# yhenon/pixeltable-yolox

Measured on AMD Instinct MI355X. Metric: images/sec (fwd+NMS) YOLOX-s 640×640 bf16 @1/2/4/8 MI355X; box mAP parity, higher is better.
Workload: dtype bf16

## Files before the change

### pixeltable-yolox_amd/csrc/conv_ws.hip

```cpp
#include "conv_common.hpp"
#include "lds_dma.hpp"

#ifndef YXH_WS_PROBE
#define YXH_WS_PROBE 0
#endif

#ifndef YXH_WS_PD8
#define YXH_WS_PD8 0
#endif

#ifndef YXH_WS_NPIN
#define YXH_WS_NPIN 48
#endif

#ifndef YXH_WS_ACT_CT
#define YXH_WS_ACT_CT 1
#endif

namespace yxh {

namespace {

template <typename T, int CR>
__device__ __forceinline__ uint4 ws_weight_padk(const ConvParams& p, int n_first, int tap, int kb, int lane) {
    const int frow = lane & 15, fq = lane >> 4;
    const int ch = kb * 32 + fq * 8;
    if (ch >= CR) return make_uint4(0, 0, 0, 0);
    const int n = min(n_first + frow, p.cout - 1);
    return *(const uint4*)((const T*)p.w + ((long long)n * 9 + tap) * CR + ch);
}

__device__ __forceinline__ void pin_agpr(uint4& v) {
    typedef unsigned u32x4v __attribute__((ext_vector_type(4)));
    u32x4v t = {v.x, v.y, v.z, v.w};
    asm volatile("" : "+a"(t));
    v = make_uint4(t.x, t.y, t.z, t.w);
}

constexpr int ws_ps(int c16, int s) {
    return s == 1 ? c16 + (6 - c16 % 4) % 4 : (c16 % 2 ? c16 : c16 + 1);
}
constexpr int ws_hxp(int tx, int s) {
    const int hx = (tx - 1) * s + 3;
    if (tx % 16 == 0) return hx;
    int h = hx;
    while (h % 8 != tx % 8) ++h;
    return h;
}

}

template <typename T, int CIN, int S, int TX, int TY, int TN, int WN, int WK, int WM, int BPC, bool F1, int PGN = 0,
          int PGC = 0, int PGH = 0, int CR = CIN, bool A32 = false>
__global__ __launch_bounds__(64 * WN * WK * WM, BPC) void conv_ws(ConvParams p, int tiles_x, int tiles_y,
                                                                 int ntiles, int ntn, int nwork) {
    static_assert(sizeof(T) == 2, "16-bit operands");
    constexpr int NW = WN * WK * WM;
    constexpr int NCB = CIN / 32, WCB = NCB / WK;
    constexpr int WTN = TN / WN, FR = WTN / 16;
    constexpr int TM = TX * TY, WTM = TM / WM, FC = WTM / 16;
    constexpr int HX = (TX - 1) * S + 3, HY = (TY - 1) * S + 3, HXP = ws_hxp(TX, S);
    constexpr int C16 = CIN / 8, PS = ws_ps(C16, S), PSB = PS * 16;
    constexpr int SLOTS = HY * HXP * PS, LOADS = (SLOTS + 63) / 64, GB = (LOADS + NW - 1) / NW;
    constexpr int RBYTES = WK > 1 ? WN * WM * FR * FC * (WK - 1) * 1024 : 0;
    constexpr bool PG = PGN > 0, HP = PGH > 0, PGY = PG || HP;
    constexpr int RS = TN / 8 + 1, RSLOTS = (S == 1 || PGY) ? TM * RS : 0;
    constexpr int RLOADS = (RSLOTS + 63) / 64, GR = (RLOADS + NW - 1) / NW, RTB = RLOADS * 1024;
    constexpr int NRING = 3;
    constexpr int XS = PGC / 8 + 1, XSLOTS = PG && PGC > 0 ? TM * XS : 0;
    constexpr int XLOADS = (XSLOTS + 63) / 64, GX = (XLOADS + NW - 1) / NW, XTB = XLOADS * 1024;
    constexpr int K2 = TN + PGC, KB2 = K2 / 32;
    constexpr int WN2 = PG ? (NW < PGN / 16 ? NW : PGN / 16) : 1, WM2 = NW / WN2;
    constexpr int NF2 = PG ? PGN / 16 / WN2 : 1, PF2 = TM / 16 / WM2;
    static_assert(!PG || (!F1 && TN % 32 == 0 && PGC % 32 == 0 && PGN % (16 * WN2) == 0 &&
                          NW % WN2 == 0 && (TM / 16) % WM2 == 0), "post-conv tile");
    static_assert(!HP || (!PG && !F1 && S == 1 && TN % 32 == 0), "head-form tile");
    constexpr int HROWS = HP ? PGH * 16 : 0, HBYTES_W = HROWS * RS * 16 + HROWS * 4;
    constexpr int NG = CIN / 32, R1 = NW / NG, NPA = (HY * HXP + 15) / 16;
    constexpr int HBYTES = LOADS * 1024;
    constexpr int XOFF = 2 * HBYTES + RBYTES + NRING * RTB;
    constexpr int TOFF = XOFF + 3 * XTB;
    constexpr int HWOFF = TOFF + (F1 ? HBYTES : 0);
    constexpr int SMEM = HWOFF + HBYTES_W;
    static_assert(!F1 || (S == 1 && NW % NG == 0), "fused Bottleneck tile");
    constexpr int FCO = (FC + WK - 1) / WK;
    constexpr int NS = WCB * 9;
    constexpr int PD = YXH_WS_PD8 && FR * FC >= 8 ? YXH_WS_PD8 : FR * FC >= 8 ? 1 : FR * FC >= 4 ? 2 : 3;
    static_assert(NCB % WK == 0 && WTN % 16 == 0 && WTM % 16 == 0 && TM % (16 * WM) == 0, "tile");
    static_assert(FR * 9 * WCB * 4 <= (NW == 4 && BPC == 1 ? 288 : 160), "weights must stay in VGPRs");
    static_assert(SMEM <= 160 * 1024 && SMEM * BPC <= 160 * 1024, "LDS (BPC blocks per CU must fit)");
    constexpr int NPIN = !F1 && FR * 9 * WCB * 4 > 160 ? YXH_WS_NPIN : 0;
    __shared__ __attribute__((aligned(16))) char smem[SMEM];

    const int tid = threadIdx.x, lane = tid & 63;
    const int wave = __builtin_amdgcn_readfirstlane(tid >> 6);
    const int wn = wave % WN, wk = (wave / WN) % WK, wm = wave / (WN * WK);
    const int frow = lane & 15, fq = lane >> 4;
    const int bid = dma::xcd_remap(blockIdx.x, gridDim.x);
    const int nt = bid % ntn, worker = bid / ntn;
    const int n0 = nt * TN;
    const int tile = worker;
    if (tile >= ntiles) return;

    const int cin_ = p.cin, cout = p.cout, in_w = p.in_w, in_h = p.in_h, scs = p.scs[0];
    const int OH = p.out_h, OW = p.out_w, ohw = p.ohw;
    (void)cin_;

    uint32_t boff[FC];
#pragma unroll
    for (int j = 0; j < FC; ++j) {
        const int pl = (wm * FC + j) * 16 + frow;
        const int ty = pl / TX, tx = pl - ty * TX;
        boff[j] = (uint32_t)((ty * S * HXP + tx * S) * PSB + (wk * WCB * 4 + fq) * 16);
    }

    const uint32_t lds0 = dma::lds_addr(smem);
    const uint32_t bytes = (uint32_t)((long long)in_h * in_w * scs * 2);
    const int gsrc = p.grp2 && n0 >= cout / 2 ? CR : 0;

    int hrel[GB], hyx[GB];
#pragma unroll
    for (int i = 0; i < GB; ++i) {
        const int L = wave + NW * i;
        const int s = 64 * L + lane;
        const int hp = s / PS, c16 = s - hp * PS;
        const int hy = hp / HXP, hx = hp - hy * HXP;
        const bool st = L < LOADS && s < SLOTS && c16 < CR / 8 && hx < HX;
        hyx[i] = st ? (hy | (hx << 16)) : 0x7fff7fff;
        hrel[i] = ((hy * in_w + hx) * scs + c16 * 8) * 2;
    }

    struct TileC { int b, oy0, ox0; };
    const unsigned txy = (unsigned)(tiles_x * tiles_y);
    auto coords = [&](int t) -> TileC {
        const unsigned b = (unsigned)t / txy, r = (unsigned)t - b * txy;
        const unsigned ty = r / (unsigned)tiles_x, tx = r - ty * (unsigned)tiles_x;
        return TileC{(int)b, (int)ty * TY, (int)tx * TX};
    };

    auto issue_halo = [&](const TileC& c, int kb) {
        const int iy0 = c.oy0 * S - 1, ix0 = c.ox0 * S - 1;
        const int base = (iy0 * in_w + ix0) * scs * 2;
        const dma::u32x4 rsrc = dma::srd((const T*)p.sptr[0] + (long long)c.b * p.sbs[0] + gsrc, bytes);
#pragma unroll
        for (int i = 0; i < GB; ++i) {
            const int L = wave + NW * i;
            if (LOADS % NW == 0 || i + 1 < GB || L < LOADS) {
                const int iy = iy0 + (hyx[i] & 0xffff), ix = ix0 + (hyx[i] >> 16);
                const bool ok = (unsigned)iy < (unsigned)in_h && (unsigned)ix < (unsigned)in_w;
                const uint32_t voff = ok ? (uint32_t)(base + hrel[i]) : dma::kOob;
                dma::load16(rsrc, voff, 0u, __builtin_amdgcn_readfirstlane(lds0 + (uint32_t)(kb * HBYTES + L * 1024)));
            }
        }
    };

    const bool silu = p.act == YXH_ACT_SILU;
    const bool has_res = p.res != nullptr;
    const bool pg_store = PG && p.pg_store;
    const uint32_t dbytes = (uint32_t)((long long)ohw * p.dst_cs * (A32 ? 4 : 2));
    const uint32_t rbytes = (uint32_t)((long long)ohw * p.res_cs * 2);
    const int dcs = p.dst_cs, rcs = p.res_cs;
    const uint32_t res_lds = lds0 + (uint32_t)(2 * HBYTES + RBYTES);

    int rgeo[GR > 0 ? GR : 1];
#pragma unroll
    for (int i = 0; i < GR; ++i) {
        const int L = wave + NW * i;
        const int sl = 64 * L + lane;
        const int pl = sl / RS, ch = sl - pl * RS;
        const int ty = pl / TX, tx = pl - ty * TX;
        const bool st = L < RLOADS && sl < RSLOTS && ch < TN / 8 && n0 + ch * 8 < cout;
        rgeo[i] = st ? (ty | (tx << 10) | (ch << 20)) : -1;
    }
    auto issue_res = [&](const TileC& c, int slot) {
        if constexpr (GR > 0) {
            const dma::u32x4 rsrc = dma::srd((const T*)p.res + (long long)c.b * p.res_bs, rbytes);
#pragma unroll
            for (int i = 0; i < GR; ++i) {
                const int L = wave + NW * i;
                if (RLOADS % NW == 0 || i + 1 < GR || L < RLOADS) {
                    const int g = rgeo[i];
                    const int oy = c.oy0 + (g & 1023), ox = c.ox0 + ((g >> 10) & 1023);
                    const bool ok = g >= 0 && oy < OH && ox < OW;
                    const uint32_t voff = ok ? (uint32_t)(((oy * OW + ox) * rcs + n0 + (g >> 20) * 8) * 2) : dma::kOob;
                    dma::load16(rsrc, voff, 0u, __builtin_amdgcn_readfirstlane(res_lds + (uint32_t)(slot * RTB + L * 1024)));
                }
            }
        }
    };

    int xgeo[GX > 0 ? GX : 1];
#pragma unroll
    for (int i = 0; i < GX; ++i) {
        const int L = wave + NW * i;
        const int sl = 64 * L + lane;
        const int pl = sl / XS, ch = sl - pl * XS;
        const int ty = pl / TX, tx = pl - ty * TX;
        const bool st = L < XLOADS && sl < XSLOTS && ch < PGC / 8;
        xgeo[i] = st ? (ty | (tx << 10) | (ch << 20)) : -1;
    }
    auto issue_x2 = [&](const TileC& c, int slot) {
        if constexpr (GX > 0) {
            const dma::u32x4 xsrc =
                dma::srd((const T*)p.pgs + (long long)c.b * p.pgs_bs, (uint32_t)((long long)ohw * p.pgs_cs * 2));
#pragma unroll
            for (int i = 0; i < GX; ++i) {
                const int L = wave + NW * i;
                if (XLOADS % NW == 0 || i + 1 < GX || L < XLOADS) {
                    const int g = xgeo[i];
                    const int oy = c.oy0 + (g & 1023), ox = c.ox0 + ((g >> 10) & 1023);
                    const bool ok = g >= 0 && oy < OH && ox < OW;
                    const uint32_t voff = ok ? (uint32_t)(((oy * OW + ox) * p.pgs_cs + (g >> 20) * 8) * 2) : dma::kOob;
                    dma::load16(xsrc, voff, 0u,
                                __builtin_amdgcn_readfirstlane(lds0 + (uint32_t)(XOFF + slot * XTB + L * 1024)));
                }
            }
        }
    };

    TileC cur = coords(tile), cnext{0, 0, 0}, prev{0, 0, 0}, prev2{0, 0, 0};
    issue_halo(cur, 0);
    if (!PGY && has_res) issue_res(cur, 0);
    if (tile + nwork < ntiles) {
        cnext = coords(tile + nwork);
        issue_halo(cnext, 1);
        if (!PGY && has_res) issue_res(cnext, 1);
    }

    const bool hgrp1 = HP && n0 >= cout / 2;
    const int hrows = HP ? (hgrp1 ? p.pg_cout2 : p.pg_cout) : 0;

    uint4 a1[F1 ? 2 : 1][F1 ? NG : 1];
    float b1[2][4];
    if constexpr (F1) {
        const T* w1 = (const T*)p.pw1;
        const int g = wave % NG;
#pragma unroll
        for (int i = 0; i < 2; ++i) {
#pragma unroll
            for (int cb = 0; cb < NG; ++cb)
                a1[i][cb] = *(const uint4*)(w1 + (g * 32 + i * 16 + frow) * CIN + cb * 32 + fq * 8);
#pragma unroll
            for (int r = 0; r < 4; ++r) b1[i][r] = p.pb1[g * 32 + i * 16 + fq * 4 + r];
        }
    }

    uint4 a[FR][9][WCB];
#pragma unroll
    for (int c = 0; c < WCB; ++c)
#pragma unroll
        for (int tap = 0; tap < 9; ++tap)
#pragma unroll
            for (int i = 0; i < FR; ++i)
                a[i][tap][c] = CR == CIN ? ws_weight<T>(p, n0 + wn * WTN + i * 16, tap, 9, CIN, wk * WCB + c, lane)
                                         : ws_weight_padk<T, CR>(p, n0 + wn * WTN + i * 16, tap, wk * WCB + c, lane);
    float bias[FR][4];
#pragma unroll
    for (int i = 0; i < FR; ++i) {
        const int n = n0 + wn * WTN + i * 16 + fq * 4;
#pragma unroll
        for (int r = 0; r < 4; ++r) bias[i][r] = n + r < cout ? p.bias[n + r] : 0.0f;
    }


    const int wn2 = wave % WN2, wm2 = wave / WN2;
    uint4 a2[PG ? NF2 : 1][PG ? KB2 : 1];
    float b2[PG ? NF2 : 1][4];
    if constexpr (PG) {
        const T* w2 = (const T*)p.pgw;
#pragma unroll
        for (int f = 0; f < NF2; ++f) {
            const int n = (wn2 * NF2 + f) * 16;
#pragma unroll
            for (int kb = 0; kb < KB2; ++kb) a2[f][kb] = *(const uint4*)(w2 + (long long)(n + frow) * K2 + kb * 32 + fq * 8);
#pragma unroll
            for (int r = 0; r < 4; ++r) b2[f][r] = p.pgb[n + fq * 4 + r];
        }
    }

    typedef uint32_t u32x2 __attribute__((ext_vector_type(2)));
    struct EpiCtx { __amdgpu_buffer_rsrc_t dsrd; const char* rl; TileC c; };
    auto epi_ctx = [&](const TileC c, const int k) -> EpiCtx {
        char* db = (char*)p.dst + (long long)c.b * p.dst_bs * (A32 ? 4 : 2);
        return EpiCtx{__builtin_amdgcn_make_buffer_rsrc((void*)db, (short)0, (int)dbytes, 0x00020000),
                      smem + 2 * HBYTES + RBYTES + (k % NRING) * RTB, c};
    };
    auto epi_piece = [&](const EpiCtx& e, const f32x4 (&ap)[FR][FCO], const int o, const int i, auto act_c) {
        constexpr int AC = decltype(act_c)::value;
        const int j = wk + WK * o;
        const int pl = (wm * FC + j) * 16 + frow;
        const int ty = pl / TX, tx = pl - ty * TX;
        const int oy = e.c.oy0 + ty, ox = e.c.ox0 + tx;
        const int nl = wn * WTN + i * 16 + fq * 4, n = n0 + nl;
        const bool ok = j < FC && oy < OH && ox < OW && n < cout;
        if constexpr (A32) {
            typedef uint32_t u32x4 __attribute__((ext_vector_type(4)));
            const int od4 = ok ? ((oy * OW + ox) * dcs + n) * 4 : (int)dma::kOob;
            f32x4 v = ap[i][o] + f32x4{bias[i][0], bias[i][1], bias[i][2], bias[i][3]};
            if (p.accum) v += __builtin_bit_cast(f32x4, __builtin_amdgcn_raw_buffer_load_b128(e.dsrd, od4, 0, 0));
            __builtin_amdgcn_raw_buffer_store_b128(__builtin_bit_cast(u32x4, v), e.dsrd, od4, 0, 0);
            return;
        }
        const int od = ok ? ((oy * OW + ox) * dcs + n) * 2 : (int)dma::kOob;
        u32x2 rv = {0u, 0u};
        if constexpr (GR > 0) rv = *(const u32x2*)(e.rl + (pl * RS + (nl >> 3)) * 16 + (nl & 7) * 2);
        T rt[4];
        __builtin_memcpy(rt, &rv, 8);
        const f32x4 x = ap[i][o] + f32x4{bias[i][0], bias[i][1], bias[i][2], bias[i][3]};
        f32x4 v;
        if constexpr (AC == 1) v = yxh::silu4(x);
        else if constexpr (AC == 2) v = x;
        else v = silu ? yxh::silu4(x) : x;
        if (has_res) v = v + f32x4{to_f32(rt[0]), to_f32(rt[1]), to_f32(rt[2]), to_f32(rt[3])};
        T t[4] = {from_f32<T>(v[0]), from_f32<T>(v[1]), from_f32<T>(v[2]), from_f32<T>(v[3])};
        u32x2 u;
        __builtin_memcpy(&u, t, 8);
        if constexpr (PGY) {
            *(u32x2*)(e.rl + (pl * RS + (nl >> 3)) * 16 + (nl & 7) * 2) = u;
            if (PG && pg_store) __builtin_amdgcn_raw_buffer_store_b64(u, e.dsrd, od, 0, 0);
        } else if (!(YXH_WS_PROBE & 1) || p.act == 12345) {
            __builtin_amdgcn_raw_buffer_store_b64(u, e.dsrd, od, 0, 0);
        }
    };
    auto epilogue = [&](const TileC c, const int k, const f32x4 (&ap)[FR][FCO], auto act_c) {
        const EpiCtx e = epi_ctx(c, k);
#pragma unroll
        for (int o = 0; o < FCO; ++o)
#pragma unroll
            for (int i = 0; i < FR; ++i) epi_piece(e, ap, o, i, act_c);
    };

    struct PostCtx { __amdgpu_buffer_rsrc_t srd; const char* ys; const char* xs; TileC c; };
    auto post_ctx = [&](const TileC c, const int k) -> PostCtx {
        PostCtx q;
        q.c = c;
        q.ys = smem + 2 * HBYTES + RBYTES + (k % NRING) * RTB;
        q.xs = smem + XOFF + (k % 3) * XTB;
        const int es = HP ? 4 : 2;
        q.srd = __builtin_amdgcn_make_buffer_rsrc((void*)((char*)p.pgd + (long long)c.b * p.pgd_bs * es), (short)0,
                                                  (int)((long long)ohw * p.pgd_cs * es), 0x00020000);
        return q;
    };
    constexpr int HPF = (TM / 16 + NW - 1) / NW;
    constexpr int NPU = PG ? PF2 * NF2 : HP ? HPF * PGH : 0;
    constexpr int KBP = PG ? KB2 : HP ? 2 * (TN / 32) : 1;
    constexpr bool SPLIT = PG;
    constexpr int SP = SPLIT && NS / (NPU + 1) > 1 ? NS / (NPU + 1) : 1;
    auto post_skip = [&](const int u) -> bool {
        if constexpr (HP) {
            const int pf = wave + NW * (u / PGH), f = u - PGH * (u / PGH);
            return pf >= TM / 16 || f >= (hgrp1 ? 1 : PGH);
        }
        return false;
    };
    auto post_load = [&](const PostCtx& q, const int u, uint4 (&ob)[KBP]) {
        if constexpr (PG) {
            const int pf = u / NF2;
            const int pl = (wm2 * PF2 + pf) * 16 + frow;
#pragma unroll
            for (int kb = 0; kb < KB2; ++kb)
                ob[kb] = kb < TN / 32 ? *(const uint4*)(q.ys + (pl * RS + kb * 4 + fq) * 16)
                                      : *(const uint4*)(q.xs + (pl * XS + (kb - TN / 32) * 4 + fq) * 16);
        } else if constexpr (HP) {
            if (post_skip(u)) return;
            const int pf = wave + NW * (u / PGH), f = u - PGH * (u / PGH);
            const char* wl = smem + HWOFF;
#pragma unroll
            for (int kb = 0; kb < TN / 32; ++kb) {
                ob[2 * kb] = *(const uint4*)(q.ys + ((pf * 16 + frow) * RS + kb * 4 + fq) * 16);
                ob[2 * kb + 1] = *(const uint4*)(wl + ((f * 16 + frow) * RS + kb * 4 + fq) * 16);
            }
        }
    };
    auto post_math = [&](const PostCtx& q, const int u, const uint4 (&ob)[KBP]) {
        if constexpr (PG) {
            const int pf = u / NF2, f = u - NF2 * (u / NF2);
            const int pl = (wm2 * PF2 + pf) * 16 + frow;
            f32x4 z = f32x4{0.f, 0.f, 0.f, 0.f};
#pragma unroll
            for (int kb = 0; kb < KB2; ++kb) Mma<T>::run(z, a2[f][kb], ob[kb]);
            const int ty = pl / TX, tx = pl - ty * TX;
            const int oy = q.c.oy0 + ty, ox = q.c.ox0 + tx;
            const int n = (wn2 * NF2 + f) * 16 + fq * 4;
            const f32x4 zs = yxh::silu4(z + f32x4{b2[f][0], b2[f][1], b2[f][2], b2[f][3]});
            T t[4] = {from_f32<T>(zs[0]), from_f32<T>(zs[1]), from_f32<T>(zs[2]), from_f32<T>(zs[3])};
            u32x2 uv;
            __builtin_memcpy(&uv, t, 8);
            const int od = oy < OH && ox < OW ? ((oy * OW + ox) * p.pgd_cs + n) * 2 : (int)dma::kOob;
            __builtin_amdgcn_raw_buffer_store_b64(uv, q.srd, od, 0, 0);
        } else if constexpr (HP) {
            if (post_skip(u)) return;
            const int pf = wave + NW * (u / PGH), f = u - PGH * (u / PGH);
            const float* bl = (const float*)(smem + HWOFF + HROWS * RS * 16);
            f32x4 z = f32x4{0.f, 0.f, 0.f, 0.f};
#pragma unroll
            for (int kb = 0; kb < TN / 32; ++kb) Mma<T>::run(z, ob[2 * kb], ob[2 * kb + 1]);
            const float st = p.pg_stride;
            const int ch = f * 16 + frow;
            const float bch = bl[ch];
#pragma unroll
            for (int r = 0; r < 4; ++r) {
                const int pl = pf * 16 + fq * 4 + r;
                const int ty = pl / TX, tx = pl - ty * TX;
                const int oy = q.c.oy0 + ty, ox = q.c.ox0 + tx;
                const bool okp = oy < OH && ox < OW;
                const int rowo = (oy * OW + ox) * p.pgd_cs + (hgrp1 ? 0 : 5);
                float v = z[r] + bch;
                if (hgrp1) {
                    if (ch < 2) v = (v + (float)(ch == 0 ? ox : oy)) * st;
                    else if (ch < 4) v = __builtin_amdgcn_exp2f(v * 1.4426950408889634f) * st;
                    else v = __builtin_amdgcn_rcpf(1.0f + __builtin_amdgcn_exp2f(-v * 1.4426950408889634f));
                } else {
                    v = __builtin_amdgcn_rcpf(1.0f + __builtin_amdgcn_exp2f(-v * 1.4426950408889634f));
                }
                __builtin_amdgcn_raw_buffer_store_b32(__float_as_uint(v), q.srd,
                                                      okp && ch < hrows ? (rowo + ch) * 4 : (int)dma::kOob, 0, 0);
            }
        }
    };
    auto post_piece = [&](const PostCtx& q, const int u) {
        uint4 ob[KBP];
        post_load(q, u, ob);
        post_math(q, u, ob);
    };
    auto post_all = [&](const PostCtx& q) {
#pragma unroll
        for (int u = 0; u < NPU; ++u) post_piece(q, u);
    };

    f32x4 accp[FR][FCO];
    constexpr int NP = FR * FCO;

    auto tile_step = [&](const TileC cur, const int tile, const int k, TileC& cnext, const TileC prev,
                         const TileC prev2, auto epi, auto post, auto first, auto act_c) -> int {
        constexpr bool EPI = decltype(epi)::value;
        constexpr bool POST = decltype(post)::value && PGY;
        constexpr bool FIRST = decltype(first)::value;
        const int kb = k & 1;
        const int next = tile + nwork;
        if constexpr (FIRST) dma::wait_vm<(FR * 9 * WCB < 63 ? FR * 9 * WCB : 63)>();
        else dma::wait_vm<0>();
        dma::barrier();
        if (next < ntiles) {
            cnext = coords(next);
            if (!FIRST && !(YXH_WS_PROBE & 2)) {
                issue_halo(cnext, kb ^ 1);
                if (!PGY && has_res) issue_res(cnext, (k + 1) % 3);
            }
        }
        if constexpr (PGY) {
            if (has_res) issue_res(cur, k % 3);
            issue_x2(cur, k % 3);
        }

        if constexpr (F1) {
            const char* hx_img = smem + kb * HBYTES;
            char* timg = smem + TOFF;
            const int g = wave % NG;
            for (int fa = wave / NG; fa < NPA; fa += R1) {
                const int hq = fa * 16 + frow;
                const int hpr = min(hq, HY * HXP - 1);
                f32x4 t2[2] = {f32x4{0.f, 0.f, 0.f, 0.f}, f32x4{0.f, 0.f, 0.f, 0.f}};
#pragma unroll
                for (int cb = 0; cb < NG; ++cb) {
                    const uint4 xb = *(const uint4*)(hx_img + hpr * PSB + (cb * 4 + fq) * 16);
                    Mma<T>::run(t2[0], a1[0][cb], xb);
                    Mma<T>::run(t2[1], a1[1][cb], xb);
                }
                const int hy = hq / HXP, hx = hq - hy * HXP;
                const int iy = cur.oy0 - 1 + hy, ix = cur.ox0 - 1 + hx;
                const bool valid = hx < HX && (unsigned)iy < (unsigned)in_h && (unsigned)ix < (unsigned)in_w;
#pragma unroll
                for (int i = 0; i < 2; ++i) {
                    T t[4];
#pragma unroll
                    for (int q = 0; q < 4; ++q) {
                        const float x = t2[i][q] + b1[i][q];
                        t[q] = from_f32<T>(valid ? (silu ? yxh::silu<false>(x) : x) : 0.0f);
                    }
                    u32x2 u;
                    __builtin_memcpy(&u, t, 8);
                    if (hq < HY * HXP) *(u32x2*)(timg + hq * PSB + (g * 32 + i * 16 + fq * 4) * 2) = u;
                }
            }
            dma::barrier();
        }

        f32x4 acc[FR][FC];
#pragma unroll
        for (int i = 0; i < FR; ++i)
#pragma unroll
            for (int j = 0; j < FC; ++j) acc[i][j] = f32x4{0.f, 0.f, 0.f, 0.f};
        const char* hb = F1 ? smem + TOFF : smem + kb * HBYTES;
        uint4 bf[PD + 1][FC];
        auto load_b = [&](int s, uint4 (&d)[FC]) {
            const int c = s / 9, tap = s - 9 * (s / 9);
            const int ky = tap / 3, kx = tap - 3 * (tap / 3);
            const int so = (ky * HXP + kx) * PSB + c * 64;
#pragma unroll
            for (int j = 0; j < FC; ++j) d[j] = *(const uint4*)(hb + boff[j] + so);
        };
#pragma unroll
        for (int q = 0; q < PD; ++q)
            if (q < NS) load_b(q, bf[q]);
        __builtin_amdgcn_sched_group_barrier(0x100, FC * (PD < NS ? PD : NS), 0);
        EpiCtx e{};
        if constexpr (EPI) e = epi_ctx(prev, k - 1);
        PostCtx pc{};
        if constexpr (POST) pc = post_ctx(prev2, k - 2);
        uint4 pob[KBP];
#pragma unroll
        for (int s = 0; s < NS; ++s) {
            if (s + PD < NS) load_b(s + PD, bf[(s + PD) % (PD + 1)]);
            const int c = s / 9, tap = s - 9 * (s / 9);
            if constexpr (FIRST && NPIN > 0) {
#pragma unroll
                for (int i = 0; i < FR; ++i)
                    if ((c * 9 + tap) * FR + i < NPIN) pin_agpr(a[i][tap][c]);
            }
            if constexpr (HP) {
#pragma unroll
                for (int i = 0; i < FR; ++i)
#pragma unroll
                    for (int j = 0; j < FC; ++j) Mma<T>::run(acc[i][j], a[i][tap][c], bf[s % (PD + 1)][j]);
            } else {
#pragma unroll
                for (int j = 0; j < FC; ++j)
#pragma unroll
                    for (int i = 0; i < FR; ++i) Mma<T>::run(acc[i][j], a[i][tap][c], bf[s % (PD + 1)][j]);
            }
            if constexpr (EPI)
                if (s < NP) epi_piece(e, accp, s / FR, s % FR, act_c);
            if constexpr (POST && SPLIT) {
                if (s >= 1 && (s - 1) % SP == 0 && (s - 1) / SP < NPU) post_math(pc, (s - 1) / SP, pob);
                if (s % SP == 0 && s / SP < NPU) post_load(pc, s / SP, pob);
            } else if constexpr (POST) {
                if (s % SP == 0 && s / SP < NPU) post_piece(pc, s / SP);
            }
            if (s + PD < NS) __builtin_amdgcn_sched_group_barrier(0x100, FC, 0);
#pragma unroll
            for (int m = 0; m < FR * FC; ++m) {
                __builtin_amdgcn_sched_group_barrier(0x008, 1, 0);
                if constexpr (EPI) __builtin_amdgcn_sched_group_barrier(0x002, 2, 0);
            }
        }
        if constexpr (EPI)
#pragma unroll
            for (int q = NS; q < NP; ++q) epi_piece(e, accp, q / FR, q % FR, act_c);
        if constexpr (POST) {
            if (SPLIT && (NS - 1) % SP == 0 && (NS - 1) / SP < NPU) post_math(pc, (NS - 1) / SP, pob);
#pragma unroll
            for (int u = (NS + SP - 1) / SP; u < NPU; ++u) post_piece(pc, u);
        }

        if constexpr (WK > 1) {
            char* red = smem + 2 * HBYTES;
            const int grp = wm * WN + wn;
#pragma unroll
            for (int i = 0; i < FR; ++i)
#pragma unroll
                for (int j = 0; j < FC; ++j) {
                    const int own = j % WK;
                    if (own != wk) {
                        const int slot = wk < own ? wk : wk - 1;
                        *(f32x4*)(red + (((grp * FR + i) * FC + j) * (WK - 1) + slot) * 1024 + lane * 16) = acc[i][j];
                    }
                }
            dma::barrier();
#pragma unroll
            for (int i = 0; i < FR; ++i)
#pragma unroll
                for (int j = 0; j < FC; ++j)
                    if (j % WK == wk) {
                        f32x4 v = acc[i][j];
#pragma unroll
                        for (int o = 0; o < WK - 1; ++o)
                            v += *(const f32x4*)(red + (((grp * FR + i) * FC + j) * (WK - 1) + o) * 1024 + lane * 16);
                        accp[i][j / WK] = v;
                    }
        } else {
#pragma unroll
            for (int i = 0; i < FR; ++i)
#pragma unroll
                for (int j = 0; j < FC; ++j) accp[i][j] = acc[i][j];
        }
        return next;
    };

    using act_rt = std::integral_constant<int, 0>;
    int next = tile_step(cur, tile, 0, cnext, cur, cur, std::false_type{}, std::false_type{}, std::true_type{}, act_rt{});
    if constexpr (HP) {
        const T* hw = (const T*)(hgrp1 ? p.pgw2 : p.pgw);
        const float* hb = hgrp1 ? p.pgb2 : p.pgb;
        char* wl = smem + HWOFF;
        for (int q = tid; q < HROWS * (TN / 8); q += 64 * NW) {
            const int r = q / (TN / 8), c = q - (TN / 8) * (q / (TN / 8));
            *(uint4*)(wl + (r * RS + c) * 16) = r < hrows ? *(const uint4*)(hw + (long long)r * TN + c * 8)
                                                          : make_uint4(0, 0, 0, 0);
        }
        for (int q = tid; q < HROWS; q += 64 * NW) ((float*)(wl + HROWS * RS * 16))[q] = q < hrows ? hb[q] : 0.0f;
    }

    constexpr bool ACT_CT = YXH_WS_ACT_CT && !A32 && !PGY && !F1 && NW == 4 && BPC == 1;
    if constexpr (ACT_CT) {
        auto tile_loop = [&](auto act_c) {
            int k = 1;
            for (; next < ntiles; ++k) {
                prev2 = prev;
                prev = cur;
                cur = cnext;
                next = tile_step(cur, next, k, cnext, prev, prev2, std::true_type{}, std::false_type{}, std::false_type{},
                                 act_c);
            }
            epilogue(cur, k - 1, accp, act_c);
        };
        if (silu) tile_loop(std::integral_constant<int, 1>{});
        else tile_loop(std::integral_constant<int, 2>{});
    } else {
        int k = 1;
        for (; next < ntiles; ++k) {
            prev2 = prev;
            prev = cur;
            cur = cnext;
            if (PGY && k >= 2)
                next = tile_step(cur, next, k, cnext, prev, prev2, std::true_type{}, std::integral_constant<bool, PGY>{},
                                 std::false_type{}, act_rt{});
            else
                next = tile_step(cur, next, k, cnext, prev, prev2, std::true_type{}, std::false_type{}, std::false_type{},
                                 act_rt{});
        }
        if constexpr (PGY) {
            dma::wait_vm<0>();
            dma::barrier();
            if (k >= 2) post_all(post_ctx(prev, k - 2));
        }
        epilogue(cur, k - 1, accp, act_rt{});
        if constexpr (PGY) {
            dma::barrier();
            post_all(post_ctx(cur, k - 1));
        }
    }
    (void)ohw;
}

template <typename T, int CIN, int S, int TX, int TY, int TN, int WN, int WK, int WM, int BPC = 1, bool F1 = false,
          int PGN = 0, int PGC = 0, int PGH = 0, int CR = CIN, bool A32 = false>
static int launch_ws(const ConvParams& p, hipStream_t st) {
    if (p.stride != S || p.cin != CR) {
        set_error("conv_ws variant built for stride %d, %d input channels", S, CR);
        return YXH_EUNSUPPORTED;
    }
    if (CR != CIN && (p.grp2 || PGN > 0 || PGH > 0 || F1 || p.scs[0] % 8 || (uintptr_t)p.sptr[0] % 16)) {
        set_error("conv_ws padded-K variant (%d -> %d channels): plain conv over 16-byte pixel rows only", CR, CIN);
        return YXH_EUNSUPPORTED;
    }
    if (PGH > 0) {
        if (!p.grp2 || !p.pgw2 || p.cout != 2 * TN || (p.pg_cout + 15) / 16 != PGH) {
            set_error("conv_ws head-form tile: two groups of %d channels, %d class fragments", TN, PGH);
            return YXH_EUNSUPPORTED;
        }
    } else if ((p.pgw != nullptr) != (PGN > 0) || p.pgw2 || (p.pg_store && PGN == 0) ||
               (PGN > 0 && (p.pg_cout != PGN || p.pgs_ch != PGC || p.cout != TN))) {
        set_error(PGN > 0 ? "conv_ws post tile built for %d -> %d channels + a %d-channel post_src, post conv %d"
                          : "conv_ws plain tile with a post conv (%d -> %d, %d, %d)",
                  CIN, TN, PGC, PGN);
        return YXH_EUNSUPPORTED;
    }
    if (p.grp2 && (F1 || PGN > 0 || (p.cout / 2) % TN)) {
        set_error("conv_ws variant (%d input channels) cannot split its channel tiles over two groups", CIN);
        return YXH_EUNSUPPORTED;
    }
    if ((p.pw1 != nullptr) != F1) {
        set_error(F1 ? "conv_ws fused-Bottleneck variant (%d input channels) needs pre_weight"
                     : "conv_ws plain variant (%d input channels) with a pre_weight",
                  CIN);
        return YXH_EUNSUPPORTED;
    }
    if (A32) {
        if (!p.dst_f32 || p.act != YXH_ACT_NONE || p.res || p.grp2 || p.cout % 4 || ((uintptr_t)p.dst % 16) ||
            p.dst_cs % 4 || p.dst_bs % 4 || (long long)p.ohw * p.dst_cs * 4 >= (1LL << 31)) {
            set_error("conv_ws fp32-gradient tile: fp32 dst of 16-byte rows, no activation / residual");
            return YXH_EUNSUPPORTED;
        }
    } else if (p.dst_f32 || p.accum || (p.act != YXH_ACT_SILU && p.act != YXH_ACT_NONE) ||
        (!p.vec_store && PGN == 0 && PGH == 0) ||
        p.cout % 8 || (p.res && (S != 1 || ((uintptr_t)p.res % 16) || p.res_cs % 8 || p.res_bs % 8))) {
        set_error("conv_ws: 16-bit dst, SiLU/no activation, 8-byte aligned dst rows, 16-byte residual rows "
                  "(stride-1 variants) only");
        return YXH_EUNSUPPORTED;
    }
    const int tiles_x = (p.out_w + TX - 1) / TX, tiles_y = (p.out_h + TY - 1) / TY;
    const long long ntiles = (long long)tiles_x * tiles_y * (p.M / p.ohw);
    const int ntn = (p.cout + TN - 1) / TN;
    if (ntiles >= (1LL << 30)) {
        set_error("conv_ws: too many tiles");
        return YXH_EINVAL;
    }
    const int nwork = (int)std::min<long long>(ntiles, std::max(1, p.cus * BPC / ntn));
    hipLaunchKernelGGL((conv_ws<T, CIN, S, TX, TY, TN, WN, WK, WM, BPC, F1, PGN, PGC, PGH, CR, A32>), dim3((unsigned)(nwork * ntn)),
                       dim3(64 * WN * WK * WM), 0, st, p, tiles_x, tiles_y, (int)ntiles, ntn, nwork);
    YXH_CHECK_LAUNCH("conv_ws launch");
    return YXH_OK;
}

template <typename T>
static int ws_dispatch_t(int id, const ConvParams& p, hipStream_t st) {
    switch (id) {
        case 1: return launch_ws<T, 32, 1, 16, 8, 32, 1, 1, 4>(p, st);
        case 2: return launch_ws<T, 32, 1, 16, 16, 32, 1, 1, 8>(p, st);
        case 3: return launch_ws<T, 32, 2, 16, 8, 64, 2, 1, 4>(p, st);
        case 4: return launch_ws<T, 32, 2, 16, 4, 64, 2, 1, 2, 2>(p, st);
        case 5: return launch_ws<T, 64, 1, 16, 8, 64, 2, 1, 4>(p, st);
        case 6: return launch_ws<T, 64, 1, 16, 4, 64, 2, 1, 2, 2>(p, st);
        case 7: return launch_ws<T, 64, 2, 16, 4, 128, 4, 1, 2>(p, st);
        case 8: return launch_ws<T, 64, 2, 16, 2, 128, 4, 1, 1, 2>(p, st);
        case 11: return launch_ws<T, 128, 1, 8, 4, 128, 4, 2, 1>(p, st);
        case 12: return launch_ws<T, 128, 1, 8, 8, 64, 2, 2, 1>(p, st);
        case 13: return launch_ws<T, 128, 2, 16, 2, 128, 4, 2, 1>(p, st);
        case 14: return launch_ws<T, 128, 2, 8, 4, 128, 4, 2, 1>(p, st);
        case 15: return launch_ws<T, 128, 1, 16, 4, 64, 2, 2, 1>(p, st);
        case 16: return launch_ws<T, 256, 1, 8, 4, 64, 2, 4, 1>(p, st);
        case 17: return launch_ws<T, 256, 1, 16, 2, 64, 2, 4, 1>(p, st);
        case 18: return launch_ws<T, 32, 1, 16, 8, 32, 1, 1, 4, 2>(p, st);
        case 19: return launch_ws<T, 64, 1, 32, 2, 64, 2, 1, 2, 2>(p, st);
        case 20: return launch_ws<T, 128, 1, 16, 2, 64, 2, 2, 1, 2>(p, st);
        case 21: return launch_ws<T, 128, 1, 8, 4, 64, 2, 2, 1, 2>(p, st);
        case 22: return launch_ws<T, 128, 2, 16, 1, 64, 2, 2, 1, 2>(p, st);
        case 23: return launch_ws<T, 256, 1, 8, 2, 32, 1, 4, 1, 2>(p, st);
        case 24: return launch_ws<T, 64, 2, 16, 2, 64, 2, 1, 2, 2>(p, st);
        case 25: return launch_ws<T, 128, 1, 16, 4, 128, 4, 1, 1>(p, st);
        case 26: return launch_ws<T, 128, 1, 16, 2, 128, 4, 1, 1>(p, st);
        case 27: return launch_ws<T, 128, 1, 8, 4, 128, 4, 1, 1>(p, st);
        case 28: return launch_ws<T, 256, 2, 8, 2, 32, 1, 4, 1>(p, st);
        case 29: return launch_ws<T, 256, 2, 8, 2, 64, 2, 4, 1>(p, st);
        case 30: return launch_ws<T, 256, 2, 16, 1, 32, 1, 4, 1>(p, st);
        case 31: return launch_ws<T, 32, 1, 16, 8, 32, 1, 1, 4, 1, true>(p, st);
        case 32: return launch_ws<T, 32, 1, 16, 16, 32, 1, 1, 8, 1, true>(p, st);
        case 33: return launch_ws<T, 64, 1, 16, 4, 64, 2, 1, 2, 1, true>(p, st);
        case 34: return launch_ws<T, 64, 1, 16, 8, 64, 2, 1, 2, 1, true>(p, st);
        case 35: return launch_ws<T, 128, 1, 16, 4, 128, 4, 1, 1, 1, true>(p, st);
        case 36: return launch_ws<T, 128, 1, 8, 4, 128, 4, 1, 1, 1, true>(p, st);
        case 41: return launch_ws<T, 32, 1, 16, 8, 32, 1, 1, 4, 1, false, 64, 32>(p, st);
        case 42: return launch_ws<T, 32, 1, 16, 4, 32, 1, 1, 4, 2, false, 64, 32>(p, st);
        case 43: return launch_ws<T, 64, 1, 16, 4, 64, 2, 1, 2, 1, false, 128, 64>(p, st);
        case 44: return launch_ws<T, 64, 1, 8, 4, 64, 2, 2, 1, 2, false, 128, 64>(p, st);
        case 45: return launch_ws<T, 64, 2, 16, 2, 128, 4, 1, 1, 1, false, 128, 0>(p, st);
        case 46: return launch_ws<T, 64, 2, 16, 4, 128, 4, 1, 1, 1, false, 128, 0>(p, st);
        case 47: return launch_ws<T, 64, 1, 16, 2, 64, 2, 2, 1, 2, false, 128, 64>(p, st);
        case 48: return launch_ws<T, 64, 1, 16, 4, 64, 2, 2, 1, 1, false, 128, 64>(p, st);
        case 49: return launch_ws<T, 64, 2, 16, 2, 128, 4, 2, 1, 1, false, 128, 0>(p, st);
        case 50: return launch_ws<T, 64, 2, 8, 4, 128, 4, 2, 1, 1, false, 128, 0>(p, st);
        case 51: return launch_ws<T, 128, 1, 16, 4, 128, 4, 1, 1, 1, false, 0, 0, 5>(p, st);
        case 53: return launch_ws<T, 128, 1, 16, 2, 128, 4, 1, 1, 1, false, 0, 0, 5>(p, st);
        case 52: return launch_ws<T, 64, 1, 16, 8, 64, 2, 1, 2, 1, false, 64, 0>(p, st);
        case 54: return launch_ws<T, 64, 1, 16, 4, 64, 2, 1, 2, 1, false, 64, 0>(p, st);
        case 55: return launch_ws<T, 128, 1, 8, 4, 128, 4, 1, 1, 1, false, 128, 0>(p, st);
        case 56: return launch_ws<T, 128, 1, 16, 2, 128, 4, 1, 1, 1, false, 128, 0>(p, st);
        case 61: return launch_ws<T, 96, 1, 16, 4, 80, 5, 1, 1, 1, false, 0, 0, 0, 80>(p, st);
        case 62: return launch_ws<T, 96, 1, 16, 4, 32, 2, 1, 2, 2, false, 0, 0, 0, 80>(p, st);
        case 63: return launch_ws<T, 96, 2, 16, 4, 80, 5, 1, 1, 1, false, 0, 0, 0, 80>(p, st);
        case 64: return launch_ws<T, 96, 2, 16, 4, 32, 2, 1, 2, 1, false, 0, 0, 0, 80>(p, st);
        case 65: return launch_ws<T, 160, 1, 16, 4, 64, 4, 1, 1>(p, st);
        case 66: return launch_ws<T, 160, 1, 16, 4, 32, 2, 1, 2>(p, st);
        case 67: return launch_ws<T, 160, 2, 16, 2, 64, 4, 1, 1>(p, st);
        case 68: return launch_ws<T, 160, 2, 16, 2, 32, 2, 1, 2>(p, st);
        case 69: return launch_ws<T, 320, 1, 8, 4, 32, 2, 2, 1>(p, st);
        case 71: return launch_ws<T, 320, 1, 16, 2, 32, 2, 2, 1>(p, st);
        case 72: return launch_ws<T, 320, 2, 16, 1, 32, 2, 2, 1>(p, st);
        case 74: return launch_ws<T, 512, 1, 8, 2, 32, 2, 4, 1>(p, st);
        case 76: return launch_ws<T, 512, 1, 16, 1, 32, 2, 4, 1>(p, st);
        case 79: return launch_ws<T, 160, 1, 16, 2, 64, 4, 1, 1>(p, st);
        case 80: return launch_ws<T, 96, 1, 8, 4, 32, 2, 1, 2, 2, false, 0, 0, 0, 80>(p, st);
        case 81: return launch_ws<T, 96, 1, 16, 4, 32, 2, 1, 2, 2, false, 0, 0, 0, 80, true>(p, st);
        case 82: return launch_ws<T, 160, 1, 16, 4, 64, 4, 1, 1, 1, false, 0, 0, 0, 160, true>(p, st);
        case 83: return launch_ws<T, 160, 1, 16, 4, 32, 2, 1, 2, 1, false, 0, 0, 0, 160, true>(p, st);
        case 84: return launch_ws<T, 320, 1, 8, 4, 32, 2, 2, 1, 1, false, 0, 0, 0, 320, true>(p, st);
        case 85: return launch_ws<T, 320, 1, 16, 2, 32, 2, 2, 1, 1, false, 0, 0, 0, 320, true>(p, st);
        case 86: return launch_ws<T, 64, 1, 16, 4, 64, 2, 1, 2, 2, false, 0, 0, 0, 64, true>(p, st);
        case 87: return launch_ws<T, 128, 1, 16, 4, 128, 4, 1, 1, 1, false, 0, 0, 0, 128, true>(p, st);
        case 88: return launch_ws<T, 256, 1, 8, 4, 64, 2, 4, 1, 1, false, 0, 0, 0, 256, true>(p, st);
        case 89: return launch_ws<T, 32, 1, 16, 4, 80, 5, 1, 1, 1, false, 0, 0, 0, 16>(p, st);
        default: set_error("conv_ws tile id %d", id); return YXH_EINVAL;
    }
}

int conv_ws_dispatch(int dtype, int id, const ConvParams& p, hipStream_t st) {
    if (p.taps != 9 || p.kw != 3 || p.pad != 1 || p.nsrc != 1 || p.sup[0] || p.sw[0] != p.in_w) {
        set_error("conv_ws needs a 3x3 pad-1 conv over one plain source");
        return YXH_EUNSUPPORTED;
    }
    if ((long long)p.in_h * p.in_w * p.scs[0] * 2 >= (1LL << 31)) {
        set_error("conv_ws: image exceeds 31-bit byte offsets");
        return YXH_EUNSUPPORTED;
    }
    if (dtype == YXH_BF16) return ws_dispatch_t<bf16>(id, p, st);
    if (dtype == YXH_F16) return ws_dispatch_t<f16>(id, p, st);
    set_error("conv_ws is built for bf16/f16");
    return YXH_EUNSUPPORTED;
}

}
```

Baseline: 19760.

## Share halo LDS reads across fragments that hit the same row offset in conv_ws

Adds a compile-time read schedule that deduplicates the LDS B-fragment loads when several output fragments of a wave read the same halo position for different taps (possible when 16 is divisible by the tile width). The main loop becomes one iteration per unique read, with a ring buffer and a computed read distance, and each loaded fragment feeds every MFMA that needs it. The epilogue and post pieces are reinterleaved by MFMA count. The goal is fewer ds_read instructions and less LDS bandwidth per tap. In exchange the code is more complex, MFMA order changes, and a few tile configurations are excluded to keep the per-tap path.

```diff
diff --git a/pixeltable-yolox_amd/csrc/conv_ws.hip b/pixeltable-yolox_amd/csrc/conv_ws.hip
--- a/pixeltable-yolox_amd/csrc/conv_ws.hip
+++ b/pixeltable-yolox_amd/csrc/conv_ws.hip
@@ -7,6 +7,14 @@
 
 #ifndef YXH_WS_PD8
 #define YXH_WS_PD8 0
+#endif
+
+#ifndef YXH_WS_ROWSHARE
+#define YXH_WS_ROWSHARE 1
+#endif
+
+#ifndef YXH_WS_RD
+#define YXH_WS_RD 0
 #endif
 
 #ifndef YXH_WS_NPIN
@@ -46,6 +54,114 @@
     int h = hx;
     while (h % 8 != tx % 8) ++h;
     return h;
+}
+
+template <int S, int TX, int FC>
+struct WsSched {
+    int nrd = 0;
+    int row[FC * 9] = {}, col[FC * 9] = {};
+    int nuse[FC * 9] = {};
+    int uj[FC * 9][FC] = {}, utap[FC * 9][FC] = {};
+    int before[FC * 9 + 1] = {};
+    int jfirst[9] = {};
+};
+
+template <int S, int TX, int FC>
+constexpr WsSched<S, TX, FC> ws_sched() {
+    WsSched<S, TX, FC> s{};
+    constexpr bool SHARE = 16 % TX == 0;
+    for (int j = 0; j < FC; ++j)
+        for (int tap = 0; tap < 9; ++tap) {
+            const int row = (j * 16 / TX) * S + tap / 3, col = (j * 16 % TX) * S + tap % 3;
+            int k = 0;
+            while (k < s.nrd && (s.row[k] < row || (s.row[k] == row && s.col[k] < col))) ++k;
+            if (!(SHARE && k < s.nrd && s.row[k] == row && s.col[k] == col)) {
+                for (int q = s.nrd; q > k; --q) {
+                    s.row[q] = s.row[q - 1], s.col[q] = s.col[q - 1], s.nuse[q] = s.nuse[q - 1];
+                    for (int u = 0; u < FC; ++u) s.uj[q][u] = s.uj[q - 1][u], s.utap[q][u] = s.utap[q - 1][u];
+                }
+                s.row[k] = row, s.col[k] = col, s.nuse[k] = 0;
+                ++s.nrd;
+            }
+            s.uj[k][s.nuse[k]] = j, s.utap[k][s.nuse[k]] = tap;
+            ++s.nuse[k];
+        }
+    for (int r = 0; r < s.nrd; ++r) s.before[r + 1] = s.before[r] + s.nuse[r];
+    for (int tap = 0; tap < 9; ++tap) {
+        bool found = false;
+        for (int r = 0; r < s.nrd && !found; ++r)
+            for (int u = 0; u < s.nuse[r] && !found; ++u)
+                if (s.utap[r][u] == tap) s.jfirst[tap] = s.uj[r][u], found = true;
+    }
+    return s;
+}
+
+template <int S, int TX, int FC>
+constexpr bool ws_sched_ok(const WsSched<S, TX, FC>& s) {
+    int seen[FC][9] = {}, last[FC] = {};
+    for (int j = 0; j < FC; ++j) last[j] = -1;
+    for (int r = 0; r < s.nrd; ++r) {
+        if (s.nuse[r] < 1 || s.nuse[r] > FC) return false;
+        for (int u = 0; u < s.nuse[r]; ++u) {
+            const int j = s.uj[r][u], tap = s.utap[r][u];
+            if (j < 0 || j >= FC || tap < 0 || tap > 8 || seen[j][tap]++ || tap <= last[j]) return false;
+            last[j] = tap;
+            if ((j * 16 / TX) * S + tap / 3 != s.row[r] || (j * 16 % TX) * S + tap % 3 != s.col[r]) return false;
+        }
+    }
+    for (int j = 0; j < FC; ++j)
+        for (int tap = 0; tap < 9; ++tap)
+            if (seen[j][tap] != 1) return false;
+    return s.before[s.nrd] == FC * 9;
+}
+
+template <int S, int TX, int FC>
+struct WsSchedOf {
+    static constexpr WsSched<S, TX, FC> v = ws_sched<S, TX, FC>();
+    static_assert(ws_sched_ok(v), "conv_ws read schedule");
+};
+static_assert(WsSchedOf<1, 16, 4>::v.nrd == 18, "16-wide stride 1, four rows per wave (id 25)");
+static_assert(WsSchedOf<1, 16, 2>::v.nrd == 12, "16-wide stride 1, two rows per wave (ids 1, 5, 43, 47, 54)");
+static_assert(WsSchedOf<1, 8, 2>::v.nrd == 15, "8-wide stride 1, 8x4 pixels per wave (ids 11, 27, 44, 55)");
+static_assert(WsSchedOf<2, 16, 2>::v.nrd == 15 && WsSchedOf<2, 16, 4>::v.nrd == 27, "16-wide stride 2 (13, 49 / 46)");
+static_assert(WsSchedOf<1, 32, 2>::v.nrd == 18 && WsSchedOf<2, 8, 2>::v.nrd == 18 && WsSchedOf<1, 16, 1>::v.nrd == 9,
+              "nothing shared: 32-wide (id 19), stride-2 8x4 (id 14), one fragment per wave (id 42)");
+
+template <int S, int TX, int FC>
+constexpr int ws_read_distance(const WsSched<S, TX, FC>& s, int uses) {
+    for (int d = 1; d < s.nrd; ++d) {
+        bool ok = true;
+        for (int r = 0; r < s.nrd && ok; ++r) {
+            int n = 0;
+            for (int q = 1; q <= d; ++q) n += s.nuse[(r - q + d * s.nrd) % s.nrd];
+            ok = n >= uses;
+        }
+        if (ok) return d;
+    }
+    return s.nrd;
+}
+
+constexpr bool ws_keep_per_tap(int cin, int s, int tx, int ty, int tn, int wk, int wm, int bpc) {
+    return s == 1 && ((cin == 64 && tx == 16 && tn == 64 && wk == 1 && ((ty == 8 && wm == 4 && bpc == 1) || (ty == 4 && wm == 2 && bpc == 2))) ||
+                      (cin == 128 && tx == 8 && ty == 4 && wk == 2 && wm == 1 && ((tn == 128 && bpc == 1) || (tn == 64 && bpc == 2))));
+}
+
+constexpr int ws_ride_ds(int s0, int s1, bool epi_ds, int np, bool split, int sp, int npu, int kbp) {
+    int n = 0;
+    for (int s = s0; s < s1; ++s) {
+        if (epi_ds && s < np) ++n;
+        if (split && s % sp == 0 && s / sp < npu) n += kbp;
+    }
+    return n;
+}
+
+template <typename F, int... I>
+__device__ __forceinline__ void ws_static_for(F&& f, std::integer_sequence<int, I...>) {
+    (f(std::integral_constant<int, I>{}), ...);
+}
+template <int N, typename F>
+__device__ __forceinline__ void ws_static_for(F&& f) {
+    ws_static_for(f, std::make_integer_sequence<int, N>{});
 }
 
 }
@@ -86,6 +202,13 @@
     constexpr int FCO = (FC + WK - 1) / WK;
     constexpr int NS = WCB * 9;
     constexpr int PD = YXH_WS_PD8 && FR * FC >= 8 ? YXH_WS_PD8 : FR * FC >= 8 ? 1 : FR * FC >= 4 ? 2 : 3;
+    using Sch = WsSchedOf<S, TX, FC>;
+    constexpr int NRD = Sch::v.nrd, NR = WCB * NRD;
+    constexpr bool RSH = YXH_WS_ROWSHARE && !F1 && !HP && NRD < 9 * FC &&
+                         !(!PG && !A32 && CR == CIN && ws_keep_per_tap(CIN, S, TX, TY, TN, WK, WM, BPC));
+    constexpr int RDA = ws_read_distance(Sch::v, ((FR * FC >= 16 ? 12 : 8) + FR - 1) / FR);
+    constexpr int RD = (YXH_WS_RD ? YXH_WS_RD : RDA) < NR ? (YXH_WS_RD ? YXH_WS_RD : RDA) : NR;
+    static_assert(!RSH || (16 % TX == 0 && (FC * 16) % TX == 0), "row-shared reads need whole-row fragments");
     static_assert(NCB % WK == 0 && WTN % 16 == 0 && WTM % 16 == 0 && TM % (16 * WM) == 0, "tile");
     static_assert(FR * 9 * WCB * 4 <= (NW == 4 && BPC == 1 ? 288 : 160), "weights must stay in VGPRs");
     static_assert(SMEM <= 160 * 1024 && SMEM * BPC <= 160 * 1024, "LDS (BPC blocks per CU must fit)");
@@ -492,6 +615,56 @@
 #pragma unroll
             for (int j = 0; j < FC; ++j) acc[i][j] = f32x4{0.f, 0.f, 0.f, 0.f};
         const char* hb = F1 ? smem + TOFF : smem + kb * HBYTES;
+        EpiCtx e{};
+        PostCtx pc{};
+        uint4 pob[KBP];
+        if constexpr (RSH) {
+        constexpr int MPS = FR * FC;
+        uint4 ring[RD + 1];
+        auto load_r = [&](auto G, uint4& d) {
+            constexpr int g = decltype(G)::value, c = g / NRD, r = g - NRD * (g / NRD);
+            constexpr int so = (Sch::v.row[r] * HXP + Sch::v.col[r]) * PSB + c * 64;
+            d = *(const uint4*)(hb + boff[0] + so);
+        };
+        ws_static_for<RD>([&](auto Q) { load_r(Q, ring[decltype(Q)::value]); });
+        __builtin_amdgcn_sched_group_barrier(0x100, RD, 0);
+        if constexpr (EPI) e = epi_ctx(prev, k - 1);
+        if constexpr (POST) pc = post_ctx(prev2, k - 2);
+        ws_static_for<NR>([&](auto G) {
+            constexpr int g = decltype(G)::value, c = g / NRD, r = g - NRD * (g / NRD);
+            constexpr int NU = Sch::v.nuse[r];
+            if constexpr (g + RD < NR) load_r(std::integral_constant<int, g + RD>{}, ring[(g + RD) % (RD + 1)]);
+            ws_static_for<NU>([&](auto U) {
+                constexpr int j = Sch::v.uj[r][decltype(U)::value], tap = Sch::v.utap[r][decltype(U)::value];
+                if constexpr (FIRST && NPIN > 0 && j == Sch::v.jfirst[tap]) {
+#pragma unroll
+                    for (int i = 0; i < FR; ++i)
+                        if ((c * 9 + tap) * FR + i < NPIN) pin_agpr(a[i][tap][c]);
+                }
+#pragma unroll
+                for (int i = 0; i < FR; ++i) Mma<T>::run(acc[i][j], a[i][tap][c], ring[g % (RD + 1)]);
+            });
+            constexpr int M0 = (c * 9 * FC + Sch::v.before[r]) * FR, M1 = M0 + NU * FR;
+            constexpr int S0 = (M0 + MPS - 1) / MPS, S1 = (M1 + MPS - 1) / MPS;
+            ws_static_for<S1 - S0>([&](auto SS) {
+                constexpr int s = S0 + decltype(SS)::value;
+                if constexpr (EPI && s < NP) epi_piece(e, accp, s / FR, s % FR, act_c);
+                if constexpr (POST && SPLIT) {
+                    if constexpr (s >= 1 && (s - 1) % SP == 0 && (s - 1) / SP < NPU) post_math(pc, (s - 1) / SP, pob);
+                    if constexpr (s % SP == 0 && s / SP < NPU) post_load(pc, s / SP, pob);
+                } else if constexpr (POST) {
+                    if constexpr (s % SP == 0 && s / SP < NPU) post_piece(pc, s / SP);
+                }
+            });
+            constexpr int DSN = (g + RD < NR ? 1 : 0) + ws_ride_ds(S0, S1, EPI && GR > 0, NP, POST && SPLIT, SP, NPU, KBP);
+            if constexpr (DSN > 0) __builtin_amdgcn_sched_group_barrier(0x100, DSN, 0);
+#pragma unroll
+            for (int m = 0; m < NU * FR; ++m) {
+                __builtin_amdgcn_sched_group_barrier(0x008, 1, 0);
+                if constexpr (EPI) __builtin_amdgcn_sched_group_barrier(0x002, 2, 0);
+            }
+        });
+        } else {
         uint4 bf[PD + 1][FC];
         auto load_b = [&](int s, uint4 (&d)[FC]) {
             const int c = s / 9, tap = s - 9 * (s / 9);
@@ -504,11 +677,8 @@
         for (int q = 0; q < PD; ++q)
             if (q < NS) load_b(q, bf[q]);
         __builtin_amdgcn_sched_group_barrier(0x100, FC * (PD < NS ? PD : NS), 0);
-        EpiCtx e{};
         if constexpr (EPI) e = epi_ctx(prev, k - 1);
-        PostCtx pc{};
         if constexpr (POST) pc = post_ctx(prev2, k - 2);
-        uint4 pob[KBP];
 #pragma unroll
         for (int s = 0; s < NS; ++s) {
             if (s + PD < NS) load_b(s + PD, bf[(s + PD) % (PD + 1)]);
@@ -543,6 +713,7 @@
                 __builtin_amdgcn_sched_group_barrier(0x008, 1, 0);
                 if constexpr (EPI) __builtin_amdgcn_sched_group_barrier(0x002, 2, 0);
             }
+        }
         }
         if constexpr (EPI)
 #pragma unroll
```

New measurement: 19820 (median of 6 runs). About the same (+0.3%).
